# vovach777/llcomp

Hardware: AMD Instinct MI355X
Metric: encode+decode MPix/s on 4K RGB8, bit-exact (higher is better)
Workload: dtype int32

## Files before the change

llcomp_amd/csrc/enc_rows_asm.hpp:

```cpp
#pragma once
#include <cstdint>

namespace llcomp_mi {

#define LL_B0 "v32"
#define LL_B1 "v33"
#define LL_B "v[32:33]"
#define LL_A "v32"
#define LL_EX "v33"
#define LL_E0 "v[34:35]"
#define LL_E0L "v34"
#define LL_E0H "v35"
#define LL_E1 "v[36:37]"
#define LL_E1L "v36"
#define LL_E1H "v37"
#define LL_E2 "v[38:39]"
#define LL_E2L "v38"
#define LL_E2H "v39"
#define LL_E3 "v[40:41]"
#define LL_E3L "v40"
#define LL_E3H "v41"
#define LL_E4 "v[42:43]"
#define LL_E4L "v42"
#define LL_E4H "v43"
#define LL_E5 "v[44:45]"
#define LL_E5L "v44"
#define LL_E5H "v45"
#define LL_E6 "v[46:47]"
#define LL_E6L "v46"
#define LL_E6H "v47"
#define LL_E7 "v[48:49]"
#define LL_E7L "v48"
#define LL_E7H "v49"
#define LL_LOW "v30"
#define LL_RANGE "v31"
#define LL_LR "v[30:31]"
#define LL_R1 "v50"
#define LL_BITS "v51"
#define LL_N "v51"
#define LL_OFF "v52"
#define LL_T "v53"
#define LL_CK "v34"
#define LL_CT "v35"
#define LL_CT2 "v50"
#define LL_SX "s[36:37]"
#define LL_SA "s[38:39]"
#define LL_ST "s[40:41]"
#define LL_SW "s[42:43]"
#define LL_SB "s[44:45]"
#define LL_SU "s[46:47]"
#define LL_SM "s[56:57]"
#define LL_SC "s[40:41]"
#define LL_SD "s[48:49]"
#define LL_SE "s[50:51]"
#define LL_SR "s[52:53]"
#define LL_SRL "s52"
#define LL_SRH "s53"
#define LL_SI "s54"
#define LL_S1 "s52"
#define LL_S2 "s53"

#ifndef LLMI_ASM_VAR
#define LLMI_ASM_VAR 0
#endif
#if LLMI_ASM_VAR & 1
#define LL_C3 "3"
#else
#define LL_C3 "%[c3]"
#endif
#if LLMI_ASM_VAR & 4
#define LL_PATCH_SKIP(N)
#else
#define LL_PATCH_SKIP(N) "s_cbranch_execz .Lpatch" N "_%=\n\t"
#endif
#define LL_PATCH_END(N) ".Lpatch" N "_%=:\n\t" "s_mov_b64 exec, " LL_ST "\n\t"
#if LLMI_ASM_VAR & 2
#define LL_RENORM_SKIP(N)
#else
#define LL_RENORM_SKIP(N) "s_cbranch_execz .Lskip" N "_%=\n\t"
#endif
#define LL_SPLIT(EL)                                                                                              \
    "v_mul_u32_u24_sdwa " LL_R1 ", " EL ", " LL_RANGE " dst_sel:DWORD dst_unused:UNUSED_PAD src0_sel:BYTE_1 src1_sel:DWORD\n\t" \
    "v_lshrrev_b32_e32 " LL_R1 ", 8, " LL_R1 "\n\t"                                                               \
    "v_sub_u32_e32 " LL_RANGE ", " LL_RANGE ", " LL_R1 "\n\t"
#define LL_ONE                                          \
    "v_add_u32_e32 " LL_LOW ", " LL_LOW ", " LL_RANGE "\n\t"        \
    "v_mov_b32_e32 " LL_RANGE ", " LL_R1 "\n\t"
#define LL_RENORM(N)                                                                                               \
    "v_cmp_gt_u32_e32 vcc, %[c100], " LL_RANGE "\n\t"                                                                  \
    "s_and_saveexec_b64 " LL_SW ", vcc\n\t"                                                                        \
    LL_RENORM_SKIP(N)                                                                                              \
    "ds_write_b8_d16_hi %[wp], " LL_LOW "\n\t"                                                                         \
    "v_cmp_lt_u32_e32 vcc, %[cwrap], " LL_LOW "\n\t"                                                                   \
    "s_cbranch_vccnz .Lrare" N "_%=\n"                                                                             \
    ".Lback" N "_%=:\n\t"                                                                                          \
    "v_add_u32_e32 %[wp], 1, %[wp]\n\t"                                                                            \
    "v_lshlrev_b64 " LL_LR ", 8, " LL_LR "\n\t"                                                                     \
    "v_and_b32_e32 " LL_LOW ", 0xffffff, " LL_LOW "\n"                                                                     \
    ".Lskip" N "_%=:\n\t"                                                                                          \
    "s_mov_b64 exec, " LL_SW "\n\t"
#define LL_RARE_STUB(N)                     \
    ".Lrare" N "_%=:\n\t"                   \
    "s_getpc_b64 " LL_SR "\n\t"             \
    "s_branch .Lcarry_%=\n\t"               \
    "s_branch .Lback" N "_%=\n"
#define LL_FETCH_REST                                                                                                         \
    "v_lshlrev_b32_sdwa " LL_E1L ", " LL_C3 ", " LL_B0 " dst_sel:DWORD dst_unused:UNUSED_PAD src0_sel:DWORD src1_sel:BYTE_1\n\t"      \
    "v_lshlrev_b32_sdwa " LL_E2L ", " LL_C3 ", " LL_B0 " dst_sel:DWORD dst_unused:UNUSED_PAD src0_sel:DWORD src1_sel:BYTE_2\n\t"      \
    "v_lshlrev_b32_sdwa " LL_E3L ", " LL_C3 ", " LL_B0 " dst_sel:DWORD dst_unused:UNUSED_PAD src0_sel:DWORD src1_sel:BYTE_3\n\t"      \
    "v_lshlrev_b32_sdwa " LL_E4L ", " LL_C3 ", " LL_B1 " dst_sel:DWORD dst_unused:UNUSED_PAD src0_sel:DWORD src1_sel:BYTE_0\n\t"      \
    "ds_read_b64 " LL_E1 ", " LL_E1L "\n\t"                                                                                   \
    "ds_read_b64 " LL_E2 ", " LL_E2L "\n\t"                                                                                   \
    "ds_read_b64 " LL_E3 ", " LL_E3L "\n\t"                                                                                   \
    "ds_read_b64 " LL_E4 ", " LL_E4L "\n\t"                                                                                   \
    "v_lshlrev_b32_sdwa " LL_E5L ", " LL_C3 ", " LL_B1 " dst_sel:DWORD dst_unused:UNUSED_PAD src0_sel:DWORD src1_sel:BYTE_1\n\t"      \
    "v_lshlrev_b32_sdwa " LL_E6L ", " LL_C3 ", " LL_B1 " dst_sel:DWORD dst_unused:UNUSED_PAD src0_sel:DWORD src1_sel:BYTE_2\n\t"      \
    "v_lshlrev_b32_sdwa " LL_E7L ", " LL_C3 ", " LL_B1 " dst_sel:DWORD dst_unused:UNUSED_PAD src0_sel:DWORD src1_sel:BYTE_3\n\t"      \
    "ds_read_b64 " LL_E5 ", " LL_E5L "\n\t"                                                                                   \
    "ds_read_b64 " LL_E6 ", " LL_E6L "\n\t"                                                                                   \
    "ds_read_b64 " LL_E7 ", " LL_E7L "\n\t"

struct EncRowsExtra {
    uint32_t pend;
    uint32_t hot;
    uint32_t any_pend;
};

#define LL_SNAP 0
#include "enc_sample_asm.inc"
#undef LL_SNAP
#define LL_SNAP 1
#include "enc_sample_asm.inc"
#undef LL_SNAP

}
```

llcomp_amd/csrc/enc_sample_asm.inc:

```
#if LL_SNAP
#define LL_STATE(...)
#else
#define LL_STATE(...) __VA_ARGS__
#endif
#define LL_UNARY(K, KM1, EL, EH, N, SAVE)                  \
    LL_SPLIT(EL)                                           \
    LL_STATE("ds_write_b8 %[bank], " EL " offset:" K "\n\t") \
    "v_cmp_lt_u32_e32 vcc, " KM1 ", " LL_EX "\n\t"         \
    "s_and_b64 exec, exec, vcc\n\t"                        \
    SAVE                                                   \
    "s_cbranch_execz .Lunary_done_%=\n\t"                  \
    LL_ONE                                                 \
    LL_STATE("ds_write_b8 %[bank], " EH " offset:" K "\n\t") \
    LL_RENORM(N)
#if LL_SNAP
__device__ __forceinline__ void enc_snap_sample_asm(unsigned long long& low_range, uint32_t& wp, EncRowsExtra& x, uint32_t b0, uint32_t b1,
                                                    int res, uint32_t base) {
#else
__device__ __forceinline__ void enc_rows_sample_asm(unsigned long long& low_range, uint32_t& wp, EncRowsExtra& x, uint32_t bank,
                                                    int res, uint32_t base) {
#endif
    asm volatile(
        "s_mov_b64 " LL_SX ", exec\n\t"
        LL_STATE("ds_read2st64_b32 " LL_B ", %[bank] offset1:1\n\t")
        "s_cmp_lg_u32 %[hot], 0\n\t"
        "s_waitcnt lgkmcnt(0)\n\t"
        "v_lshlrev_b32_sdwa " LL_E0L ", " LL_C3 ", " LL_B0 " dst_sel:DWORD dst_unused:UNUSED_PAD src0_sel:DWORD src1_sel:BYTE_0\n\t"
        "ds_read_b64 " LL_E0 ", " LL_E0L "\n\t"
        "s_cbranch_scc0 .Lcold_%=\n\t"
        LL_FETCH_REST
        "s_waitcnt lgkmcnt(7)\n\t"
        "s_branch .Lzero_%=\n"
        ".Lcold_%=:\n\t"
        "s_waitcnt lgkmcnt(0)\n"
        ".Lzero_%=:\n\t"
        LL_SPLIT(LL_E0L)
        LL_STATE("ds_write_b8 %[bank], " LL_E0L "\n\t")
        "v_cmp_eq_u32_e32 vcc, 0, %[res]\n\t"
        "s_andn2_b64 " LL_SA ", exec, vcc\n\t"
        "s_and_saveexec_b64 " LL_ST ", vcc\n\t"
        LL_PATCH_SKIP("0")
        LL_ONE
        LL_STATE("ds_write_b8 %[bank], " LL_E0H "\n")
        LL_PATCH_END("0")
        LL_RENORM("0")
        "s_and_b64 exec, " LL_SA ", " LL_SA "\n\t"
        "s_cbranch_execz .Ldone_%=\n\t"
        "s_mov_b64 " LL_SB ", 0\n\t"
        "s_mov_b64 " LL_SM ", 0\n\t"
        "s_cmp_lg_u32 %[hot], 0\n\t"
        "s_cbranch_scc1 .Lhave_%=\n\t"
        LL_FETCH_REST
        ".Lhave_%=:\n\t"
        "v_sub_u32_e32 " LL_A ", 0, %[res]\n\t"
        "v_max_i32_e32 " LL_A ", %[res], " LL_A "\n\t"
        "v_ffbh_u32_e32 " LL_EX ", " LL_A "\n\t"
        "v_sub_u32_e32 " LL_EX ", 31, " LL_EX "\n\t"
        "s_waitcnt lgkmcnt(0)\n\t"
        LL_UNARY("1", "0", LL_E1L, LL_E1H, "1", "s_mov_b64 " LL_SB ", exec\n\t")
        LL_UNARY("2", "1", LL_E2L, LL_E2H, "2", "s_mov_b64 " LL_SM ", exec\n\t")
        LL_UNARY("3", "2", LL_E3L, LL_E3H, "3", "")
        "s_mov_b64 " LL_SU ", exec\n\t"
        "v_add_u32_e32 " LL_N ", -3, " LL_EX "\n\t"
        "s_mov_b32 " LL_SI ", 0\n\t"
        ".p2align 6\n"
        ".Ltail_%=:\n\t"
        LL_SPLIT(LL_E4L)
        "v_cmp_lt_u32_e32 vcc, " LL_SI ", " LL_N "\n\t"
        "s_and_b64 exec, exec, vcc\n\t"
        "s_cbranch_execz .Ltail_done_%=\n\t"
        "v_lshrrev_b32_e32 " LL_OFF ", 16, " LL_E4H "\n\t"
        "ds_read_b64 " LL_E4 ", " LL_OFF "\n\t"
        LL_ONE
        LL_RENORM("4")
        "s_add_i32 " LL_SI ", " LL_SI ", 1\n\t"
        "s_waitcnt lgkmcnt(0)\n\t"
        "s_branch .Ltail_%=\n"
        ".Ltail_done_%=:\n\t"
        "s_mov_b64 exec, " LL_SU "\n\t"
        LL_STATE("ds_write_b8 %[bank], " LL_E4L " offset:256\n")
        ".Lunary_done_%=:\n\t"
        "s_mov_b64 exec, " LL_SA "\n\t"
        LL_RENORM("5")
        "s_and_b64 exec, " LL_SB ", " LL_SB "\n\t"
        "s_cbranch_execz .Lsign_%=\n\t"
        LL_SPLIT(LL_E5L)
        LL_STATE("ds_write_b8 %[bank], " LL_E5L " offset:257\n\t")
        "v_lshl_or_b32 " LL_BITS ", " LL_A ", 1, 1\n\t"
        "v_sub_u32_e32 " LL_T ", 31, " LL_EX "\n\t"
        "v_lshlrev_b32_e32 " LL_BITS ", " LL_T ", " LL_BITS "\n\t"
        "v_add_co_u32_e32 " LL_BITS ", vcc, " LL_BITS ", " LL_BITS "\n\t"
        "s_and_saveexec_b64 " LL_ST ", vcc\n\t"
        LL_PATCH_SKIP("5")
        LL_ONE
        LL_STATE("ds_write_b8 %[bank], " LL_E5H " offset:257\n")
        LL_PATCH_END("5")
        LL_RENORM("6")
        ".p2align 6\n"
        ".Lman_%=:\n\t"
        "v_cmp_ne_u32_e32 vcc, %[sent], " LL_BITS "\n\t"
        "s_and_b64 exec, exec, vcc\n\t"
        "s_cbranch_execz .Lman_done_%=\n\t"
        "v_add_co_u32_e32 " LL_BITS ", vcc, " LL_BITS ", " LL_BITS "\n\t"
        "s_waitcnt lgkmcnt(0)\n\t"
        LL_SPLIT(LL_E6L)
        "v_lshrrev_b32_e32 " LL_OFF ", 16, " LL_E6L "\n\t"
        "s_and_saveexec_b64 " LL_ST ", vcc\n\t"
        LL_PATCH_SKIP("6")
        LL_ONE
        "v_lshrrev_b32_e32 " LL_OFF ", 16, " LL_E6H "\n"
        LL_PATCH_END("6")
        "ds_read_b64 " LL_E6 ", " LL_OFF "\n\t"
        LL_RENORM("7")
        "s_branch .Lman_%=\n"
        LL_RARE_STUB("0") LL_RARE_STUB("1") LL_RARE_STUB("2") LL_RARE_STUB("3") LL_RARE_STUB("4")
        LL_RARE_STUB("5") LL_RARE_STUB("6") LL_RARE_STUB("7") LL_RARE_STUB("8")
        ".Lcarry_%=:\n\t"
        "s_and_saveexec_b64 " LL_SC ", vcc\n\t"
        "v_add_u32_e32 " LL_CK ", -1, %[wp]\n"
        ".Lcloop_%=:\n\t"
        "v_cmp_lt_u32_e32 vcc, " LL_CK ", %[base]\n\t"
        "s_and_b64 " LL_SD ", exec, vcc\n\t"
        "s_cbranch_scc0 .Lcin_%=\n\t"
        "s_mov_b64 " LL_SE ", exec\n\t"
        "s_mov_b64 exec, " LL_SD "\n\t"
        "v_mov_b32_e32 %[pend], 1\n\t"
        "s_mov_b32 %[anyp], 1\n\t"
        "s_andn2_b64 exec, " LL_SE ", " LL_SD "\n\t"
        "s_cbranch_execz .Lcdone_%=\n"
        ".Lcin_%=:\n\t"
        "ds_read_u8 " LL_CT ", " LL_CK "\n\t"
        "s_waitcnt lgkmcnt(0)\n\t"
        "v_add_u32_e32 " LL_CT2 ", 1, " LL_CT "\n\t"
        "ds_write_b8 " LL_CK ", " LL_CT2 "\n\t"
        "v_add_u32_e32 " LL_CK ", -1, " LL_CK "\n\t"
        "v_cmp_eq_u32_e32 vcc, 0xff, " LL_CT "\n\t"
        "s_and_b64 exec, exec, vcc\n\t"
        "s_cbranch_execnz .Lcloop_%=\n"
        ".Lcdone_%=:\n\t"
        "s_mov_b64 exec, " LL_SC "\n\t"
        "v_and_b32_e32 " LL_LOW ", 0xffffff, " LL_LOW "\n\t"
        "s_add_u32 " LL_SRL ", " LL_SRL ", 4\n\t"
        "s_addc_u32 " LL_SRH ", " LL_SRH ", 0\n\t"
        "s_setpc_b64 " LL_SR "\n"
        ".Lman_done_%=:\n\t"
        "s_mov_b64 exec, " LL_SM "\n\t"
        LL_STATE("v_lshrrev_b32_e32 " LL_T ", 3, " LL_OFF "\n\t")
        LL_STATE("ds_write_b8 %[bank], " LL_T " offset:258\n")
        ".Lsign_%=:\n\t"
        "s_mov_b64 exec, " LL_SA "\n\t"
        LL_SPLIT(LL_E7L)
        LL_STATE("ds_write_b8 %[bank], " LL_E7L " offset:259\n\t")
        "v_cmp_gt_i32_e32 vcc, 0, %[res]\n\t"
        "s_and_saveexec_b64 " LL_ST ", vcc\n\t"
        LL_PATCH_SKIP("7")
        LL_ONE
        LL_STATE("ds_write_b8 %[bank], " LL_E7H " offset:259\n")
        LL_PATCH_END("7")
        LL_RENORM("8")
        ".Ldone_%=:\n\t"
        "s_bcnt1_i32_b64 " LL_S1 ", " LL_SA "\n\t"
        "s_bcnt1_i32_b64 " LL_S2 ", " LL_SX "\n\t"
        "s_lshl_b32 " LL_S1 ", " LL_S1 ", 1\n\t"
        "s_cmp_ge_u32 " LL_S1 ", " LL_S2 "\n\t"
        "s_cselect_b32 %[hot], 1, 0\n\t"
        "s_mov_b64 exec, " LL_SX "\n\t"
#if LL_SNAP
        : "+{v[30:31]}"(low_range), [wp] "+v"(wp), [pend] "+v"(x.pend), [hot] "+s"(x.hot), [anyp] "+s"(x.any_pend), "+{v32}"(b0), "+{v33}"(b1)
        : [res] "v"(res),
#else
        : "+{v[30:31]}"(low_range), [wp] "+v"(wp), [pend] "+v"(x.pend), [hot] "+s"(x.hot), [anyp] "+s"(x.any_pend)
        : [bank] "v"(bank), [res] "v"(res),
#endif
          [base] "v"(base), [c100] "s"(0x100u), [cwrap] "s"(0xFFFFFFu),
          [sent] "s"(0x80000000u), [c3] "v"(3u)
        : "vcc", "scc", "memory",
#if !LL_SNAP
          "v32", "v33",
#endif
          "v34", "v35", "v36", "v37", "v38", "v39", "v40", "v41", "v42", "v43", "v44",
          "v45", "v46", "v47", "v48", "v49", "v50", "v51", "v52", "v53", "s36", "s37", "s38", "s39", "s40", "s41", "s42", "s43",
          "s44", "s45", "s46", "s47", "s48", "s49", "s50", "s51", "s52", "s53", "s54", "s56", "s57");
}


#undef LL_STATE
#undef LL_UNARY
```

llcomp_amd/csrc/slice_kernels.hip:

```cpp
#include <algorithm>
#include <type_traits>

#include "device_common.hpp"
#include "kernels.hpp"

#ifndef LLMI_ASM_ENC
#define LLMI_ASM_ENC 1
#endif
#if LLMI_ASM_ENC
#include "enc_rows_asm.hpp"
#endif
#ifndef LLMI_ASM_DEC
#define LLMI_ASM_DEC 1
#endif
#if LLMI_ASM_DEC
#include "dec_rows_asm.hpp"
#endif

namespace llcomp_mi {

namespace {

#ifdef LLMI_CLOCK_PROBE
constexpr uint32_t kProbeSlots = 1u << 15;
// ... 9 lines not shown
        if (threadIdx.x == 0) {
            g_probe[kernel][blockIdx.x & (kProbeSlots - 1)][0] = t1 - t;
            g_probe[kernel][blockIdx.x & (kProbeSlots - 1)][1] = r1 - r;
        }
    }
};
#define LLMI_PROBE_START() ProbeStamp probe_stamp; probe_stamp.start()
#define LLMI_PROBE_STOP(kernel) probe_stamp.stop(kernel)
__device__ unsigned long long g_probe_parts[kProbeSlots][4];
struct PartClock {
    unsigned long long acc[4] = {0, 0, 0, 0}, last;
    __device__ __forceinline__ void start() { last = __builtin_amdgcn_s_memtime(); }
    __device__ __forceinline__ void lap(int part) {
        const unsigned long long now = __builtin_amdgcn_s_memtime();
        acc[part] += now - last;
        last = now;
    }
    __device__ __forceinline__ void flush() {
        if (threadIdx.x == 0)
            for (int k = 0; k < 4; ++k) g_probe_parts[blockIdx.x & (kProbeSlots - 1)][k] = acc[k];
    }
};
#define LLMI_PARTS_DECL() PartClock part_clock
#define LLMI_PARTS_START() part_clock.start()
#define LLMI_PARTS_LAP(part) part_clock.lap(part)
#define LLMI_PARTS_FLUSH() part_clock.flush()
#else
#define LLMI_PROBE_START() do {} while (0)
#define LLMI_PROBE_STOP(kernel) do {} while (0)
#define LLMI_PARTS_DECL() do {} while (0)
#define LLMI_PARTS_START() do {} while (0)
#define LLMI_PARTS_LAP(part) do {} while (0)
#define LLMI_PARTS_FLUSH() do {} while (0)
#endif

using entry_t = unsigned long long;
struct EntryTable {
    entry_t v[128];
};
constexpr EntryTable make_entries() {
    EntryTable t{};
    for (uint32_t s = 0; s < 128; ++s) t.v[s] = entry_t(entry_lo(s)) | (entry_t(entry_hi(s)) << 32);
    return t;
}
__constant__ EntryTable c_entries = make_entries();

using lds_u8_ptr = __attribute__((address_space(3))) uint8_t*;
using lds_entry_ptr = const __attribute__((address_space(3))) unsigned long long*;
__device__ __forceinline__ uint32_t lds_address(const void* p) { return uint32_t(uintptr_t((lds_u8_ptr) reinterpret_cast<const uint8_t*>(p))); }
__device__ __forceinline__ void load_table(entry_t* tab) {
    const unsigned long long rebase = (unsigned long long)lds_address(tab) * 0x0001000000010000ull;
    for (uint32_t i = threadIdx.x; i < 128; i += blockDim.x) tab[i] = c_entries.v[i] + rebase;
    __syncthreads();
}
__device__ __forceinline__ entry_t lds_entry(uint32_t address) { return *reinterpret_cast<lds_entry_ptr>(uintptr_t(address)); }

__device__ __forceinline__ void drain_vector_memory() { __builtin_amdgcn_s_waitcnt(0x0F70); }

__device__ __forceinline__ uint32_t byte_of(uint32_t w, int k) { return (w >> (8 * k)) & 0xFF; }
__device__ __forceinline__ uint32_t consume_here(uint32_t v);
template <int SLOT>
__device__ __forceinline__ uint32_t slot_state(const uint32_t* bank) {
    return byte_of(bank[SLOT >> 2], SLOT & 3);
}
template <int SLOT>
__device__ __forceinline__ void set_slot_state(uint32_t* bank, uint32_t ns) {
    constexpr int W = SLOT >> 2, SH = (SLOT & 3) * 8;
    bank[W] = (bank[W] & ~(0xFFu << SH)) | (ns << SH);
}
struct Bank {
    uint32_t w[4];
    uint8_t* lds;
};
constexpr uint32_t kRowBankWords = 3 * 2 * 64;
[[maybe_unused]] __device__ __forceinline__ constexpr uint32_t rowbank_byte(int slot) { return uint32_t(slot >> 2) * 256u + uint32_t(slot & 3); }
constexpr uint32_t kWideBankWords = 3 * 4 * 64;
__device__ __forceinline__ constexpr uint32_t widebank_byte(int slot) { return uint32_t(slot >> 1) * 256u + uint32_t(slot & 1) * 2u; }
template <int SLOT>
__device__ __forceinline__ uint32_t wide_offset(const uint32_t (&w)[4]) {
    return (SLOT & 1) ? (w[SLOT >> 1] >> 16) : (w[SLOT >> 1] & 0xFFFFu);
}
template <int SLOT, bool INLDS>
__device__ __forceinline__ void put_state(Bank& b, uint32_t ns) {
    if constexpr (INLDS) b.lds[rowbank_byte(SLOT)] = uint8_t(ns);
    else set_slot_state<SLOT>(b.w, ns & 0xFF);
}
__device__ __forceinline__ uint32_t prob_of(entry_t e) { return byte_of(uint32_t(e), 1); }
__device__ __forceinline__ uint32_t successor(entry_t e, bool bit) { return bit ? uint32_t(e >> 32) : uint32_t(e); }

struct Entries {
    entry_t e0, e1, e2, e3, e4, e5, e6, e7;
    template <int SLOT>
    __device__ __forceinline__ entry_t get() const {
        if constexpr (SLOT == 0) return e0;
        else if constexpr (SLOT == 1) return e1;
        else if constexpr (SLOT == 2) return e2;
        else if constexpr (SLOT == 3) return e3;
        else if constexpr (SLOT == 4) return e4;
        else if constexpr (SLOT == 5) return e5;
        else if constexpr (SLOT == 6) return e6;
        else return e7;
    }
};
__device__ __forceinline__ void fetch_slot0(Entries& E, const uint32_t* bank, const entry_t* tab) {
    E.e0 = tab[slot_state<0>(bank)];
}
__device__ __forceinline__ void fetch_rest(Entries& E, const uint32_t* bank, const entry_t* tab) {
    E.e1 = tab[slot_state<1>(bank)];
    E.e2 = tab[slot_state<2>(bank)];
    E.e3 = tab[slot_state<3>(bank)];
    E.e4 = tab[slot_state<4>(bank)];
    E.e5 = tab[slot_state<5>(bank)];
    E.e6 = tab[slot_state<6>(bank)];
    E.e7 = tab[slot_state<7>(bank)];
}

__device__ __forceinline__ entry_t entry_at(const entry_t*, uint32_t nx) { return lds_entry(nx >> 16); }

__device__ __forceinline__ void publish_count(unsigned long long* counters, uint32_t which, uint32_t mine) {
    if (!counters) return;
    unsigned long long live = __ballot(mine != 0);
    if (live == 0) return;
    unsigned long long sum = 0;
    const unsigned long long all = __ballot(1);
    while (live) {
        const int lane = __builtin_ctzll(live);
        sum += uint32_t(__builtin_amdgcn_readlane(mine, lane));
        live &= live - 1;
    }
    if (threadIdx.x == uint32_t(__builtin_ctzll(all))) atomicAdd(counters + which, sum);
}

constexpr int kModelSmall = 0;
constexpr int kModelLarge = 1;
constexpr std::integral_constant<int, kModelSmall> no_model{};

struct RangeEnc {
    uint32_t low;
    uint32_t range;
    uint32_t wp;
    uint32_t base;
    uint8_t* area;
    int32_t flushed;
    uint8_t* out;
    uint8_t* gout;
    uint32_t oofs;
    uint32_t ostep;
    int32_t cap;
    uint32_t shift;
    uint32_t carries;
};
constexpr int kStageBytes = 32;
constexpr int kStagePad = 16;
__device__ __forceinline__ int32_t enc_pos(const RangeEnc& e) { return e.flushed + int32_t(e.wp - e.base); }
__device__ __forceinline__ uint8_t* unit_byte(RangeEnc& e, uint32_t k) {
    return e.out + ((size_t(k >> 4) << (e.shift + 4)) + (k & 15));
}
__device__ __forceinline__ void enc_flush16(RangeEnc& e) {
    uint32_t* a = reinterpret_cast<uint32_t*>(e.area);
    uint4 v, rest;
    v.x = a[0]; v.y = a[1]; v.z = a[2]; v.w = a[3];
    rest.x = a[4]; rest.y = a[5]; rest.z = a[6]; rest.w = a[7];
    if (e.flushed + 16 <= e.cap) *reinterpret_cast<uint4*>(e.gout + e.oofs) = v;
    e.oofs += e.ostep;
    a[0] = rest.x; a[1] = rest.y; a[2] = rest.z; a[3] = rest.w;
    e.flushed += 16;
    e.wp -= 16;
}
__device__ __forceinline__ void enc_carry_back(RangeEnc& e) {
    for (int32_t k = enc_pos(e) - 1; k >= 0; --k) {
        uint32_t v;
        if (k >= e.flushed) {
            uint8_t& r = e.area[k - e.flushed];
            v = r;
            r = uint8_t(v + 1);
        } else if (k < e.cap) {
            uint8_t* g = unit_byte(e, uint32_t(k));
            if (k == e.flushed - 1) ++e.carries;
            v = *g;
            *g = uint8_t(v + 1);
        } else {
            break;
        }
        if (v != 0xFF) break;
    }
}
__device__ __forceinline__ void enc_renorm(RangeEnc& e) {
    if (e.range < 0x100) {
        asm volatile("ds_write_b8_d16_hi %0, %1" : : "v"(e.wp), "v"(e.low) : "memory");
        const bool wrapped = e.low > 0xFFFFFFu;
        if (__builtin_expect(__builtin_amdgcn_ballot_w64(wrapped) != 0, 0)) {
            if (wrapped) enc_carry_back(e);
        }
        ++e.wp;
        asm("v_lshlrev_b32_sdwa %0, %1, %2 dst_sel:DWORD dst_unused:UNUSED_PAD src0_sel:DWORD src1_sel:WORD_0"
            : "=v"(e.low) : "v"(8u), "v"(e.low));
        e.range <<= 8;
    }
}
__device__ __forceinline__ void enc_core(RangeEnc& e, uint32_t P, uint32_t m) {
    const uint32_t r1 = __umul24(e.range, P) >> 8;
    const uint32_t r0 = e.range - r1;
    e.low += r0 & m;
    asm("v_bfi_b32 %0, %1, %2, %3" : "=v"(e.range) : "v"(m), "v"(r1), "v"(r0));
    enc_renorm(e);
}
__device__ __forceinline__ uint32_t successor_m(entry_t e, uint32_t m) {
    uint32_t r;
    asm("v_bfi_b32 %0, %1, %2, %3" : "=v"(r) : "v"(m), "v"(uint32_t(e >> 32)), "v"(uint32_t(e)));
    return r;
}
__device__ __forceinline__ uint32_t enc_step_msb(RangeEnc& e, uint32_t& bits, entry_t cur) {
    uint32_t off, r1;
    unsigned long long saved_exec;
    asm("v_add_co_u32_e32 %[bits], vcc, %[bits], %[bits]\n\t"
        "v_mul_u32_u24_sdwa %[r1], %[lo], %[range] dst_sel:DWORD dst_unused:UNUSED_PAD src0_sel:BYTE_1 src1_sel:DWORD\n\t"
        "v_lshrrev_b32_e32 %[r1], 8, %[r1]\n\t"
        "v_sub_u32_e32 %[range], %[range], %[r1]\n\t"
        "v_lshrrev_b32_e32 %[off], 16, %[lo]\n\t"
        "s_and_saveexec_b64 %[save], vcc\n\t"
        "v_add_u32_e32 %[low], %[low], %[range]\n\t"
        "v_mov_b32_e32 %[range], %[r1]\n\t"
        "v_lshrrev_b32_e32 %[off], 16, %[hi]\n\t"
        "s_mov_b64 exec, %[save]"
        : [bits] "+v"(bits), [range] "+v"(e.range), [low] "+v"(e.low), [off] "=&v"(off), [r1] "=&v"(r1), [save] "=&s"(saved_exec)
        : [lo] "v"(uint32_t(cur)), [hi] "v"(uint32_t(cur >> 32))
        : "vcc");
    enc_renorm(e);
    return off;
}
template <int SLOT, bool INLDS>
__device__ __forceinline__ void enc_once_m(RangeEnc& e, Bank& bank, const Entries& E, uint32_t m) {
    enc_core(e, prob_of(E.get<SLOT>()), m);
    put_state<SLOT, INLDS>(bank, successor_m(E.get<SLOT>(), m));
}
template <int SLOT, bool INLDS>
__device__ __forceinline__ void enc_once(RangeEnc& e, Bank& bank, const Entries& E, bool bit) {
    const entry_t en = E.get<SLOT>();
    const uint32_t r1 = __umul24(e.range, prob_of(en)) >> 8;
    if constexpr (INLDS) {
        e.range -= r1;
        put_state<SLOT, true>(bank, uint32_t(en));
        if (bit) {
            asm volatile("" : "+v"(e.low));
            e.low += e.range;
            e.range = r1;
            put_state<SLOT, true>(bank, uint32_t(en >> 32));
        }
        enc_renorm(e);
    } else {
        const uint32_t r0 = e.range - r1;
        e.low += bit ? r0 : 0u;
        e.range = bit ? r1 : r0;
        const uint32_t ns = successor(en, bit);
        enc_renorm(e);
        put_state<SLOT, INLDS>(bank, ns);
    }
}

template <bool ALL, bool INLDS>
__device__ __forceinline__ void enc_residual(RangeEnc& e, Bank& bank, const entry_t* tab, int res) {
    Entries E;
    fetch_slot0(E, bank.w, tab);
    if (ALL) fetch_rest(E, bank.w, tab);
    enc_once<0, INLDS>(e, bank, E, res == 0);
    if (res != 0) {
        if (!ALL) fetch_rest(E, bank.w, tab);
        const uint32_t a = uint32_t(res < 0 ? -res : res);
        const int ex = 31 - __clz(int(a));
        enc_once<1, INLDS>(e, bank, E, ex > 0);
        if (ex > 0) {
            enc_once<2, INLDS>(e, bank, E, ex > 1);
            if (ex > 1) {
                enc_once<3, INLDS>(e, bank, E, ex > 2);
                if (ex > 2) {
                    entry_t cur = E.e4;
                    const uint32_t ones = uint32_t(ex - 3);
                    uint32_t r1 = __umul24(e.range, prob_of(cur)) >> 8;
                    e.range -= r1;
                    for (uint32_t i = 0; i < ones; ++i) {
                        cur = entry_at(tab, uint32_t(cur >> 32));
                        e.low += e.range;
                        e.range = r1;
                        enc_renorm(e);
                        r1 = __umul24(e.range, prob_of(cur)) >> 8;
                        e.range -= r1;
                    }
                    enc_renorm(e);
                    put_state<4, INLDS>(bank, uint32_t(cur));
                }
            }
            enc_once_m<5, INLDS>(e, bank, E, uint32_t(__builtin_amdgcn_sbfe(int(a), uint32_t(ex - 1), 1u)));
            if (ex > 1) {
                entry_t cur = E.e6;
                uint32_t nx;
                uint32_t bits = ((a << 1) | 1u) << (32 - ex);
                do {
                    nx = enc_step_msb(e, bits, cur);
                    cur = lds_entry(nx);
                } while (bits != 0x80000000u);
                put_state<6, INLDS>(bank, (nx - lds_address(tab)) >> 3);
            }
        }
        enc_once<7, INLDS>(e, bank, E, res < 0);
    }
}

__device__ __forceinline__ void enc_finish_and_count(RangeEnc& e, int32_t& n_bytes) {
    e.range = 0xFF; e.low += 0xFF; enc_renorm(e);
    e.range = 0xFF; enc_renorm(e);
    n_bytes = enc_pos(e);
    while (int32_t(e.wp - e.base) > 0) enc_flush16(e);
}

extern __shared__ __attribute__((aligned(32))) unsigned char dyn_lds[];
constexpr uint32_t kRowsEncTabOff = 0, kRowsEncStageOff = 1024, kRowsEncBankOff = 1024 + 16 + 32 * 64;
constexpr uint32_t kRowsEncLdsBytes = kRowsEncBankOff + 3 * 64 * 8;
[[maybe_unused]] __device__ __forceinline__ void enc_carry_back_flushed(RangeEnc& e, uint8_t* out) {
    if (e.flushed > 0 && e.flushed - 1 < e.cap) ++e.carries;
    for (int32_t k = e.flushed - 1; k >= 0; --k) {
        if (k >= e.cap) break;
        uint8_t* g = out + ((size_t(uint32_t(k) >> 4) << (e.shift + 4)) + (uint32_t(k) & 15));
        const uint32_t v = *g;
        *g = uint8_t(v + 1);
        if (v != 0xFF) break;
    }
}
template <bool LDSTAB>
__device__ __forceinline__ void clear_lds_states() {
    if constexpr (LDSTAB) {
        unsigned long long* t = reinterpret_cast<unsigned long long*>(dyn_lds);
        for (uint32_t i = threadIdx.x; i < uint32_t(kContexts); i += blockDim.x) t[i] = 0;
    }
}
template <int NCH, bool ROWS, typename SYM, bool LDSTAB = false, bool SNAP = false, bool SEG = false, bool SMALL = false>
__global__ __launch_bounds__(64, ROWS ? 8 : 1) void k_encode_slices(const Geometry g, const uint32_t lpw,
                                                      const SYM* __restrict__ sym, uint64_t* __restrict__ states,
                                                      uint8_t* __restrict__ scratch, uint32_t* __restrict__ slice_len,
                                                      uint64_t* __restrict__ group_sum, uint32_t* status, const uint64_t gpat,
                                                      unsigned long long* __restrict__ counters, const uint32_t seg_first = 0,
                                                      uint32_t* __restrict__ seg_state = nullptr) {
    static_assert(!(SNAP && (ROWS || LDSTAB)) && (SNAP || !SEG), "one kernel family at a time");
    static_assert(!SMALL || (ROWS && sizeof(SYM) == 1), "the model is a template flag only where the kernel forms the contexts");
    constexpr bool ASM = (ROWS || SNAP) && LLMI_ASM_ENC != 0;
    entry_t* tab;
    uint8_t* stage;
    uint32_t* rowbank;
    if constexpr (ASM) {
        static_assert(kStagePad == 16 && kStageBytes == 32, "kRowsEncBankOff");
#ifdef LLMI_TEST_LDS_OFFSET
        __shared__ uint32_t s_displace[4];
        if (threadIdx.x < 4) reinterpret_cast<volatile uint32_t*>(s_displace)[threadIdx.x] = gpat != 0;
#endif
        tab = reinterpret_cast<entry_t*>(dyn_lds + kRowsEncTabOff);
        stage = dyn_lds + kRowsEncStageOff;
        rowbank = reinterpret_cast<uint32_t*>(dyn_lds + kRowsEncBankOff);
        if (uint32_t(uintptr_t((lds_u8_ptr)dyn_lds)) != 0) {
            if (threadIdx.x == 0) atomicOr(status, kStInternal);
            return;
        }
    } else {
        __shared__ entry_t s_tab[128];
        __shared__ __attribute__((aligned(32))) uint8_t s_stage[kStagePad + kStageBytes * 64];
        __shared__ uint32_t s_rowbank[ROWS ? kRowBankWords : 1];
        tab = s_tab;
        stage = s_stage;
        rowbank = s_rowbank;
    }
    clear_lds_states<LDSTAB>();
    load_table(tab);
    const uint32_t id = blockIdx.x * lpw + threadIdx.x;
    if (threadIdx.x >= lpw || id >= g.n_slices) return;
    const SliceRect r = slice_rect(g, id);
    RangeEnc e;
    e.low = 0; e.range = 0xFF00;
    e.flushed = 0;
    e.area = stage + kStagePad + threadIdx.x * kStageBytes;
    e.base = uint32_t(uintptr_t((lds_u8_ptr)stage)) + kStagePad + threadIdx.x * kStageBytes;
    e.wp = e.base - 1;
    e.out = scratch + ((((size_t(id >> g.lane_shift) * (g.slice_cap >> 4)) << g.lane_shift) + (id & ((1u << g.lane_shift) - 1))) << 4);
    e.gout = scratch + (((size_t(__builtin_amdgcn_readfirstlane(id >> g.lane_shift)) * (g.slice_cap >> 4)) << g.lane_shift) << 4);
    e.oofs = (id & ((1u << g.lane_shift) - 1)) << 4;
    e.ostep = 16u << g.lane_shift;
    asm volatile("" : "+v"(e.ostep));
    e.cap = int32_t(g.slice_cap);
    e.shift = g.lane_shift;
    e.carries = 0;
    const uint32_t n_row = r.sw * (NCH ? uint32_t(NCH) : g.nch);
    const SYM* p0 = sym + lane_order_index(g, id, 0);
    const size_t GW = size_t(1) << g.lane_shift;
    const uint32_t total = n_row * r.sh;
    bool hot = false;
    LLMI_PROBE_START();

    if constexpr (SNAP) {
        const uint32_t cap = snapshot_cap(g);
        const uint32_t grp = __builtin_amdgcn_readfirstlane(id >> g.lane_shift);
        const char* const gres = reinterpret_cast<const char*>(sym) + ((size_t(grp) * cap * 2) << g.lane_shift);
        const char* const gbank = reinterpret_cast<const char*>(states) + ((size_t(grp) * cap * 8) << g.lane_shift);
        const uint32_t row = 32u << g.lane_shift;
        uint32_t lofs = (id & ((1u << g.lane_shift) - 1)) * 32u;
        asm volatile("" : "+v"(lofs));
        auto load_res = [&](uint32_t i) -> int {
            i = min(i, cap - 1);
            return *reinterpret_cast<const int16_t*>(gres + size_t(i >> 4) * row + ((i & 15u) << 1) + lofs);
        };
        auto load_bank = [&](uint32_t i) -> uint2 {
            i = min(i, cap - 1);
            return *reinterpret_cast<const uint2*>(gbank + size_t(i >> 3) * (2 * row) + ((i & 7u) << 3) + 2 * lofs);
        };
        uint32_t i = 0, end = total;
        [[maybe_unused]] uint32_t* const rec = SEG ? seg_state + size_t(id) * 16 : nullptr;
        if constexpr (SEG) {
            if (seg_first >= total) return;
            i = seg_first;
            end = min(total, seg_first + kSnapMaxSamples);
            if (seg_first) {
                const uint4 a = *reinterpret_cast<const uint4*>(rec), b = *reinterpret_cast<const uint4*>(rec + 4);
                const uint4 s0 = *reinterpret_cast<const uint4*>(rec + 8), s1 = *reinterpret_cast<const uint4*>(rec + 12);
                e.low = a.x; e.range = a.y; e.wp = e.base + a.z; e.flushed = int32_t(a.w);
                e.carries = b.x; hot = b.y != 0;
                e.oofs += (uint32_t(e.flushed) >> 4) * e.ostep;
                uint32_t* const st = reinterpret_cast<uint32_t*>(e.area);
                st[0] = s0.x; st[1] = s0.y; st[2] = s0.z; st[3] = s0.w; st[4] = s1.x; st[5] = s1.y; st[6] = s1.z; st[7] = s1.w;
            }
        }
#if LLMI_ASM_ENC
        EncRowsExtra xs{0u, 0u, 0u};
        unsigned long long low_range = e.low | ((unsigned long long)e.range << 32);
#endif
        auto code = [&](int res, uint2 bk) {
#if LLMI_ASM_ENC
            enc_snap_sample_asm(low_range, e.wp, xs, bk.x, bk.y, res, e.base);
            if (__builtin_expect(xs.any_pend != 0, 0)) {
                xs.any_pend = 0;
                if (xs.pend) enc_carry_back_flushed(e, e.out);
                xs.pend = 0;
            }
#else
            Bank bank{{bk.x, bk.y}, nullptr};
            if (hot) enc_residual<true, false>(e, bank, tab, res); else enc_residual<false, false>(e, bank, tab, res);
            hot = __builtin_amdgcn_readfirstlane(2 * __popcll(__ballot(res != 0)) >= __popcll(__ballot(true)));
#endif
        };
        const uint32_t todo = end - i, todo0 = __builtin_amdgcn_readfirstlane(todo);
        const bool same = __builtin_amdgcn_ballot_w64(todo != todo0) == 0;
        const uint32_t n_bulk = i + (same ? todo0 & ~3u : 0);
        int r0 = load_res(i), r1 = load_res(i + 1), r2 = load_res(i + 2), r3 = load_res(i + 3);
        uint2 b0 = load_bank(i), b1 = load_bank(i + 1), b2 = load_bank(i + 2), b3 = load_bank(i + 3);
#define LLMI_SNAP_SAMPLE(R, B, AHEAD)                          \
        {                                                          \
            const int rc = int(consume_here(uint32_t(R)));        \
            uint2 bc = B;                                          \
            bc.x = consume_here(bc.x);                             \
            R = load_res(i + AHEAD);                               \
            B = load_bank(i + AHEAD);                              \
            if (e.wp >= e.base + 16) enc_flush16(e);               \
            code(rc, bc);                                          \
        }
        for (; i < n_bulk; i += 4) {
            LLMI_SNAP_SAMPLE(r0, b0, 4)
            LLMI_SNAP_SAMPLE(r1, b1, 5)
            LLMI_SNAP_SAMPLE(r2, b2, 6)
            LLMI_SNAP_SAMPLE(r3, b3, 7)
        }
        for (; i < end; ++i) {
            LLMI_SNAP_SAMPLE(r0, b0, 4)
            {
                const int tr = r0;
                const uint2 tb = b0;
                r0 = r1; r1 = r2; r2 = r3; r3 = tr;
                b0 = b1; b1 = b2; b2 = b3; b3 = tb;
            }
        }
#undef LLMI_SNAP_SAMPLE
#if LLMI_ASM_ENC
        e.low = uint32_t(low_range);
        e.range = uint32_t(low_range >> 32);
#endif
        if constexpr (SEG) {
            if (end < total) {
                const uint32_t* const st = reinterpret_cast<const uint32_t*>(e.area);
                *reinterpret_cast<uint4*>(rec) = make_uint4(e.low, e.range, e.wp - e.base, uint32_t(e.flushed));
                *reinterpret_cast<uint4*>(rec + 4) = make_uint4(e.carries, hot ? 1u : 0u, 0u, 0u);
                *reinterpret_cast<uint4*>(rec + 8) = make_uint4(st[0], st[1], st[2], st[3]);
                *reinterpret_cast<uint4*>(rec + 12) = make_uint4(st[4], st[5], st[6], st[7]);
                return;
            }
        }
    } else if constexpr (ROWS) {
        for (uint32_t k = 0; k < 6; ++k) rowbank[k * 64 + threadIdx.x] = 0;
        constexpr bool PX = sizeof(SYM) == 1;
        const char* gsym;
        uint32_t sofs, sstep;
        [[maybe_unused]] uint32_t n_dword = total;
        [[maybe_unused]] uint32_t psh = 0, msub = 0, my = 0;
        [[maybe_unused]] int pl = 128, pL = 128;
        if constexpr (PX) {
            const uint32_t C = g.c;
            const unsigned long long tbase = ((unsigned long long)(r.frame) * g.h + r.y0) * g.w * C + (unsigned long long)(r.x0) * C;
            const unsigned long long wbase = (unsigned long long)uint32_t(__builtin_amdgcn_readfirstlane(uint32_t(tbase))) |
                                             ((unsigned long long)uint32_t(__builtin_amdgcn_readfirstlane(uint32_t(tbase >> 32))) << 32);
            gsym = reinterpret_cast<const char*>(sym) + wbase;
            sofs = uint32_t(tbase - wbase);
            sstep = C;
            const unsigned long long total_bytes = (unsigned long long)(g.frames) * g.h * g.w * C;
            n_dword = rows_px_dwords(tbase, total, C, total_bytes);
            psh = 8 * r.ch;
            msub = C >= 3 && (r.ch == 0 || r.ch == 2) ? ~0u : 0u;
            my = C >= 3 && r.ch == 1 ? ~0u : 0u;
            asm volatile("" : "+v"(psh), "+v"(msub), "+v"(my));
        } else {
            const uint32_t grp = __builtin_amdgcn_readfirstlane(id >> g.lane_shift);
            gsym = reinterpret_cast<const char*>(sym + ((size_t(grp) * g.slice_samples) << g.lane_shift));
            sofs = (id & ((1u << g.lane_shift) - 1)) * uint32_t(sizeof(SYM));
            sstep = uint32_t(sizeof(SYM)) << g.lane_shift;
        }
        asm volatile("" : "+v"(sstep));
        auto load_sym = [&](uint32_t ofs) -> uint32_t {
            if constexpr (PX) {
                uint32_t w;
                __builtin_memcpy(&w, gsym + ofs, 4);
                return w;
            } else {
                return *reinterpret_cast<const SYM*>(gsym + ofs);
            }
        };
        auto load_at = [&](uint32_t ofs, uint32_t k) -> uint32_t {
            if constexpr (PX) {
                if (k >= n_dword) {
                    const uint8_t* p = reinterpret_cast<const uint8_t*>(gsym + ofs);
                    uint32_t w = p[0];
                    if (g.c > 1) w |= uint32_t(p[1]) << 8;
                    if (g.c > 2) w |= uint32_t(p[2]) << 16;
                    if (g.c > 3) w |= uint32_t(p[3]) << 24;
                    return w;
                }
            }
            return load_sym(ofs);
        };
        uint32_t s0 = load_at(sofs, 0);
        sofs += sstep;
        uint32_t s1 = total > 1 ? load_at(sofs, 1) : 0;
        sofs += sstep;
        uint32_t bank_base = uint32_t(uintptr_t((lds_u8_ptr) reinterpret_cast<uint8_t*>(rowbank))) + threadIdx.x * 4;
        asm volatile("" : "+v"(bank_base));
#if LLMI_ASM_ENC
        EncRowsExtra xs{0u, 0u, 0u};
        unsigned long long low_range = e.low | ((unsigned long long)e.range << 32);
#endif
        auto front = [&](uint32_t sy) -> uint32_t {
            uint32_t t = sy;
            if constexpr (PX) {
                const uint32_t G = (sy >> 8) & 0xFF;
                const int sum = int(sy & 0xFF) + int((sy >> 16) & 0xFF) - 2 * int(G);
                const int q = (sum + int((uint32_t(sum) >> 31) * 3u)) >> 2;
                t = uint32_t(int(__builtin_amdgcn_ubfe(sy, psh, 8)) - int(G & msub) + (q & int(my)));
            }
            asm volatile("" : "+v"(t) : : "memory");
            return t;
        };
        struct Ctx {
            uint32_t bofs;
            int sg;
        };
        auto context = [&](auto model) -> Ctx {
            constexpr int MODEL = decltype(model)::value;
            Ctx c{0u, 0};
            if constexpr (PX && MODEL != kModelSmall) {
                const int dq = pL - pl;
                c.sg = dq >> 31;
                asm volatile("" : "+v"(c.sg));
                const uint32_t aq = uint32_t((dq ^ c.sg) - c.sg);
                c.bofs = ((aq + 511u) & 0x200u) + ((aq + 508u) & 0x200u);
                asm volatile("" : "+v"(c.bofs));
            }
            return c;
        };
        auto code = [&](uint32_t sy, Ctx c, auto model) {
            constexpr int MODEL = decltype(model)::value;
            uint32_t bofs = c.bofs;
            int res;
            if constexpr (PX) {
                const int v = int(sy);
                res = MODEL == kModelSmall ? v - pl : ((v - pl) ^ c.sg) - c.sg;
                pL = pl;
                pl = v;
            } else if constexpr (sizeof(SYM) == 2) {
                bofs = (sy >> 3) & 0x600u;
                res = int(sy << 20) >> 20;
            } else {
                bofs = (((sy & 0xFFFF) * 109u) >> 7) & 0x600u;
                res = int(sy) >> 16;
            }
#if LLMI_ASM_ENC
            enc_rows_sample_asm(low_range, e.wp, xs, bank_base + bofs, res, e.base);
            if (__builtin_expect(xs.any_pend != 0, 0)) {
                xs.any_pend = 0;
                if (xs.pend) enc_carry_back_flushed(e, e.gout + (size_t(id & ((1u << g.lane_shift) - 1)) << 4));
                xs.pend = 0;
            }
#else
            uint32_t* bp = reinterpret_cast<uint32_t*>(reinterpret_cast<uint8_t*>(rowbank) + threadIdx.x * 4 + bofs);
            Bank bank{{bp[0], bp[64]}, reinterpret_cast<uint8_t*>(bp)};
            if (hot) enc_residual<true, true>(e, bank, tab, res); else enc_residual<false, true>(e, bank, tab, res);
            hot = __builtin_amdgcn_readfirstlane(2 * __popcll(__ballot(res != 0)) >= __popcll(__ballot(true)));
#endif
        };
        const uint32_t total0 = __builtin_amdgcn_readfirstlane(total);
        const bool same = __builtin_amdgcn_ballot_w64(total != total0) == 0;
        const uint32_t tail = PX ? rows_px_tail(g.c) : 2u;
        const uint32_t n_bulk = same && total0 > tail ? total0 - tail : 0;
        auto sample_tested = [&](uint32_t i, auto model) {
            s0 = consume_here(s0);
            const Ctx c0 = context(model);
            const uint32_t t0 = front(s0);
            const uint32_t s2 = i + 2 < total ? load_at(sofs, i + 2) : 0;
            sofs += sstep;
            if (e.wp >= e.base + 16) enc_flush16(e);
            code(t0, c0, model);
            s0 = s1;
            s1 = s2;
        };
        auto bulk = [&](uint32_t& i, auto model) {
            for (; i + 1 < n_bulk; i += 2) {
                s0 = consume_here(s0);
                const Ctx c0 = context(model);
                const uint32_t t0 = front(s0);
                s0 = load_sym(sofs);
                sofs += sstep;
                if (e.wp >= e.base + 16) enc_flush16(e);
                code(t0, c0, model);
                s1 = consume_here(s1);
                const Ctx c1 = context(model);
                const uint32_t t1 = front(s1);
                s1 = load_sym(sofs);
                sofs += sstep;
                if (e.wp >= e.base + 16) enc_flush16(e);
                code(t1, c1, model);
            }
            for (; i < total; ++i) sample_tested(i, model);
        };
        sample_tested(0, no_model);
        if (total > 1) sample_tested(1, no_model);
#if LLMI_ASM_ENC
        xs.hot = __builtin_amdgcn_readfirstlane(xs.hot);
        xs.any_pend = 0;
#endif
        uint32_t i = 2;
        bulk(i, std::integral_constant<int, SMALL ? kModelSmall : kModelLarge>{});
#if LLMI_ASM_ENC
        e.low = uint32_t(low_range);
        e.range = uint32_t(low_range >> 32);
#endif
    } else {
        uint64_t* banks;
        uint32_t bsh;
        if constexpr (LDSTAB) {
            banks = reinterpret_cast<uint64_t*>(dyn_lds);
            bsh = 0;
        } else {
            banks = states + ((size_t(id >> g.lane_shift) * kContexts) << g.lane_shift) + (id & ((1u << g.lane_shift) - 1));
            bsh = g.lane_shift;
        }
        uint32_t fk = 0;
        auto fetch = [&]() -> uint32_t { return p0[size_t(fk++) * GW]; };
        uint32_t s0 = fetch();
        uint32_t s1 = total > 1 ? fetch() : 0;
        uint64_t b0 = bank_fresh<LDSTAB>(banks[size_t(s0 & 0xFFFF) << bsh], gpat);
        for (uint32_t i = 0; i < total; ++i) {
            const uint32_t s2 = i + 2 < total ? fetch() : 0;
            const uint32_t ctx0 = s0 & 0xFFFF, ctx1 = s1 & 0xFFFF;
            const int res = int(s0) >> 16;
            uint64_t raw1 = (i + 1 < total) ? banks[size_t(ctx1) << bsh] : 0;
            Bank bank{{uint32_t(b0), uint32_t(b0 >> 32)}, nullptr};
            if (hot) enc_residual<true, false>(e, bank, tab, res); else enc_residual<false, false>(e, bank, tab, res);
            hot = __builtin_amdgcn_readfirstlane(2 * __popcll(__ballot(res != 0)) >= __popcll(__ballot(true)));
            b0 = uint64_t(bank.w[0]) | (uint64_t(bank.w[1]) << 32);
            if constexpr (!LDSTAB) drain_vector_memory();
            uint64_t b1 = bank_fresh<LDSTAB>(raw1, gpat);
            banks[size_t(ctx0) << bsh] = bank_tagged<LDSTAB>(b0, gpat);
            if (ctx1 == ctx0) b1 = b0;
            b0 = b1;
            if (e.wp >= e.base + 16) enc_flush16(e);
            s0 = s1;
            s1 = s2;
        }
    }
    int32_t n_bytes = enc_pos(e);
    enc_finish_and_count(e, n_bytes);
    LLMI_PROBE_STOP(0);
    if (n_bytes > e.cap) {
        atomicOr(status, kStOverflow);
        n_bytes = e.cap;
    }
    slice_len[id] = uint32_t(n_bytes);
    publish_count(counters, kCtrEncCarryBacks, e.carries);
    if (group_sum) {
        unsigned long long live = __ballot(1), sum = 0;
        while (live) {
            const int lane = __builtin_ctzll(live);
            sum += uint32_t(__builtin_amdgcn_readlane(n_bytes, lane));
            live &= live - 1;
        }
        if (threadIdx.x == 0) group_sum[blockIdx.x] = sum;
    }
}

template <int SLOT, bool INLDS>
__device__ __forceinline__ void dec_put_state(Bank& b, uint32_t half) {
    if constexpr (INLDS) *reinterpret_cast<uint16_t*>(b.lds + widebank_byte(SLOT)) = uint16_t(half >> 16);
    else set_slot_state<SLOT>(b.w, half & 0xFF);
}
template <int SLOT, bool INLDS>
__device__ __forceinline__ entry_t dec_entry(const Bank& b, const entry_t* tab) {
    if constexpr (INLDS) return lds_entry(wide_offset<SLOT>(b.w));
    else return tab[slot_state<SLOT>(b.w)];
}
template <bool INLDS>
__device__ __forceinline__ void dec_fetch_slot0(Entries& E, const Bank& b, const entry_t* tab) { E.e0 = dec_entry<0, INLDS>(b, tab); }
template <bool INLDS>
__device__ __forceinline__ void dec_fetch_rest(Entries& E, const Bank& b, const entry_t* tab) {
    E.e1 = dec_entry<1, INLDS>(b, tab);
    E.e2 = dec_entry<2, INLDS>(b, tab);
    E.e3 = dec_entry<3, INLDS>(b, tab);
    E.e4 = dec_entry<4, INLDS>(b, tab);
    E.e5 = dec_entry<5, INLDS>(b, tab);
    E.e6 = dec_entry<6, INLDS>(b, tab);
    E.e7 = dec_entry<7, INLDS>(b, tab);
}
struct RangeDec {
    uint32_t low, range;
    unsigned long long win;
    uint32_t nxt;
    const char* gbase;
    uint32_t ofs;
    uint32_t step;
    uint32_t ofs_end;
    uint32_t replays;
};
__device__ __forceinline__ bool window_low(const RangeDec& d) { return uint32_t(d.win >> 32) == 0; }
__device__ __forceinline__ void dec_prefetch(RangeDec& d) {
    d.nxt = *reinterpret_cast<const uint32_t*>(d.gbase + min(d.ofs, d.ofs_end));
    d.ofs += d.step;
}
__device__ __forceinline__ uint32_t consume_here(uint32_t v) {
    asm volatile("" : "+v"(v) : : "memory");
    return v;
}
__device__ __forceinline__ void dec_append(RangeDec& d) {
    const uint32_t ready = consume_here(d.nxt);
    const uint32_t sh = 31u - uint32_t(__builtin_clz(uint32_t(d.win)));
    const uint32_t rest = uint32_t(d.win) ^ (1u << sh);
    d.win = ((0x100000000ull | ready) << sh) | rest;
    dec_prefetch(d);
}
__device__ __forceinline__ void dec_append_drained(RangeDec& d) {
    dec_append(d);
    drain_vector_memory();
}
__device__ __forceinline__ void dec_open(RangeDec& d, const uint32_t* group, uint32_t lane, uint32_t shift, uint32_t len) {
    d.gbase = reinterpret_cast<const char*>(group);
    d.ofs = lane * 4;
    d.step = 4u << shift;
    asm volatile("" : "+v"(d.step));
    d.ofs_end = lane * 4 + ((len + 3) >> 2) * d.step;
    dec_prefetch(d);
    const uint32_t first = d.nxt;
    dec_prefetch(d);
    const unsigned long long both = first | ((unsigned long long)d.nxt << 32);
    dec_prefetch(d);
    d.range = 0xFF00;
    d.low = ((first & 0xFF) << 8) | ((first >> 8) & 0xFF);
    d.win = (both >> 16) | (1ull << 48);
    d.replays = 0;
}
__device__ __forceinline__ unsigned long long window_next(unsigned long long w) {
    unsigned long long r;
    asm("v_lshrrev_b64 %0, 8, %1" : "=v"(r) : "v"(w));
    return r;
}
__device__ __forceinline__ void dec_refill(RangeDec& d) {
    if (d.range < 0x100) {
        d.range <<= 8;
        d.low = (d.low << 8) | (uint32_t(d.win) & 0xFF);
        d.win = window_next(d.win);
    }
}
template <bool CHECKED>
__device__ __forceinline__ bool dec_core(RangeDec& d, uint32_t P) {
    if (CHECKED && d.win <= 1) dec_append_drained(d);
    const uint32_t r1 = __umul24(d.range, P) >> 8;
    const uint32_t r0 = d.range - r1;
    uint32_t diff;
    const bool under = __builtin_usub_overflow(d.low, r0, &diff);
    const bool bit = !under;
    d.low = under ? d.low : diff;
    d.range = under ? r0 : r1;
    dec_refill(d);
    return bit;
}
template <bool CHECKED>
__device__ __forceinline__ uint32_t dec_step_acc(RangeDec& d, uint32_t P, entry_t cur, uint32_t& w) {
    if (CHECKED && d.win <= 1) dec_append_drained(d);
    const uint32_t r1 = __umul24(d.range, P) >> 8;
    const uint32_t r0 = d.range - r1;
    uint32_t diff, nx;
    asm("v_sub_co_u32_e32 %[diff], vcc, %[low], %[r0]\n\t"
        "s_nop 1\n\t"
        "v_cndmask_b32_e32 %[range], %[r1], %[r0], vcc\n\t"
        "v_cndmask_b32_e32 %[low], %[diff], %[low], vcc\n\t"
        "v_cndmask_b32_e32 %[nx], %[hi], %[lo], vcc\n\t"
        "v_addc_co_u32_e32 %[w], vcc, %[w], %[w], vcc"
        : [diff] "=&v"(diff), [range] "=&v"(d.range), [low] "+v"(d.low), [nx] "=&v"(nx), [w] "+v"(w)
        : [r0] "v"(r0), [r1] "v"(r1), [lo] "v"(uint32_t(cur)), [hi] "v"(uint32_t(cur >> 32))
        : "vcc");
    if (d.range < 0x100) {
        d.range <<= 8;
        d.low = (d.low << 8) | (uint32_t(d.win) & 0xFF);
        d.win = window_next(d.win);
    }
    return nx;
}
template <int SLOT, bool CHECKED, bool INLDS>
__device__ __forceinline__ bool dec_once(RangeDec& d, Bank& bank, const Entries& E) {
    const entry_t en = E.get<SLOT>();
    const bool bit = dec_core<CHECKED>(d, prob_of(en));
    dec_put_state<SLOT, INLDS>(bank, successor(en, bit));
    return bit;
}
template <bool ALL, bool CHECKED, bool INLDS>
__device__ __forceinline__ bool dec_residual(RangeDec& d, Bank& bank, const entry_t* tab, uint32_t& out) {
    Entries E;
    dec_fetch_slot0<INLDS>(E, bank, tab);
    if (ALL) dec_fetch_rest<INLDS>(E, bank, tab);
    if (dec_once<0, CHECKED, INLDS>(d, bank, E)) {
        out = 0;
        return true;
    }
    if (!ALL) dec_fetch_rest<INLDS>(E, bank, tab);
    int ex = 0;
    bool ok = true;
    if (dec_once<1, CHECKED, INLDS>(d, bank, E)) {
// ... 531 lines not shown
```

Before: 28820.

## Use v_cmpx loop tests, batch staging flushes, and dot4 pixel transform

Replaces the cmp+s_and exec-narrowing pairs with single v_cmpx instructions and rotates the tail and mantissa loops so the test sits at the bottom. Batches the per-sample 16-byte staging flush behind a wave-uniform ballot with a higher threshold, so the flush branch is skipped most of the time, and adds a final flush at finish. Rewrites the RGB colour-decorrelation front end with udot4 instructions in place of several shifts and subtracts. The batched flush relies on the staging buffer having room for the extra bytes, which the new static_asserts check.

```diff
diff --git a/llcomp_amd/csrc/enc_rows_asm.hpp b/llcomp_amd/csrc/enc_rows_asm.hpp
--- a/llcomp_amd/csrc/enc_rows_asm.hpp
+++ b/llcomp_amd/csrc/enc_rows_asm.hpp
@@ -79,6 +79,7 @@
 #else
 #define LL_RENORM_SKIP(N) "s_cbranch_execz .Lskip" N "_%=\n\t"
 #endif
+#define LL_NARROW(OP, A, B) "v_cmpx_" OP "_e32 vcc, " A ", " B "\n\t"
 #define LL_SPLIT(EL)                                                                                              \
     "v_mul_u32_u24_sdwa " LL_R1 ", " EL ", " LL_RANGE " dst_sel:DWORD dst_unused:UNUSED_PAD src0_sel:BYTE_1 src1_sel:DWORD\n\t" \
     "v_lshrrev_b32_e32 " LL_R1 ", 8, " LL_R1 "\n\t"                                                               \
diff --git a/llcomp_amd/csrc/enc_sample_asm.inc b/llcomp_amd/csrc/enc_sample_asm.inc
--- a/llcomp_amd/csrc/enc_sample_asm.inc
+++ b/llcomp_amd/csrc/enc_sample_asm.inc
@@ -6,8 +6,7 @@
 #define LL_UNARY(K, KM1, EL, EH, N, SAVE)                  \
     LL_SPLIT(EL)                                           \
     LL_STATE("ds_write_b8 %[bank], " EL " offset:" K "\n\t") \
-    "v_cmp_lt_u32_e32 vcc, " KM1 ", " LL_EX "\n\t"         \
-    "s_and_b64 exec, exec, vcc\n\t"                        \
+    LL_NARROW("lt_u32", KM1, LL_EX)                        \
     SAVE                                                   \
     "s_cbranch_execz .Lunary_done_%=\n\t"                  \
     LL_ONE                                                 \
@@ -63,19 +62,20 @@
         "s_mov_b64 " LL_SU ", exec\n\t"
         "v_add_u32_e32 " LL_N ", -3, " LL_EX "\n\t"
         "s_mov_b32 " LL_SI ", 0\n\t"
+        LL_SPLIT(LL_E4L)
+        LL_NARROW("lt_u32", LL_SI, LL_N)
+        "s_cbranch_execz .Ltail_done_%=\n\t"
         ".p2align 6\n"
         ".Ltail_%=:\n\t"
-        LL_SPLIT(LL_E4L)
-        "v_cmp_lt_u32_e32 vcc, " LL_SI ", " LL_N "\n\t"
-        "s_and_b64 exec, exec, vcc\n\t"
-        "s_cbranch_execz .Ltail_done_%=\n\t"
         "v_lshrrev_b32_e32 " LL_OFF ", 16, " LL_E4H "\n\t"
         "ds_read_b64 " LL_E4 ", " LL_OFF "\n\t"
         LL_ONE
         LL_RENORM("4")
         "s_add_i32 " LL_SI ", " LL_SI ", 1\n\t"
         "s_waitcnt lgkmcnt(0)\n\t"
-        "s_branch .Ltail_%=\n"
+        LL_SPLIT(LL_E4L)
+        LL_NARROW("lt_u32", LL_SI, LL_N)
+        "s_cbranch_execnz .Ltail_%=\n"
         ".Ltail_done_%=:\n\t"
         "s_mov_b64 exec, " LL_SU "\n\t"
         LL_STATE("ds_write_b8 %[bank], " LL_E4L " offset:256\n")
@@ -96,11 +96,10 @@
         LL_STATE("ds_write_b8 %[bank], " LL_E5H " offset:257\n")
         LL_PATCH_END("5")
         LL_RENORM("6")
+        LL_NARROW("ne_u32", "%[sent]", LL_BITS)
+        "s_cbranch_execz .Lman_done_%=\n\t"
         ".p2align 6\n"
         ".Lman_%=:\n\t"
-        "v_cmp_ne_u32_e32 vcc, %[sent], " LL_BITS "\n\t"
-        "s_and_b64 exec, exec, vcc\n\t"
-        "s_cbranch_execz .Lman_done_%=\n\t"
         "v_add_co_u32_e32 " LL_BITS ", vcc, " LL_BITS ", " LL_BITS "\n\t"
         "s_waitcnt lgkmcnt(0)\n\t"
         LL_SPLIT(LL_E6L)
@@ -112,7 +111,9 @@
         LL_PATCH_END("6")
         "ds_read_b64 " LL_E6 ", " LL_OFF "\n\t"
         LL_RENORM("7")
-        "s_branch .Lman_%=\n"
+        LL_NARROW("ne_u32", "%[sent]", LL_BITS)
+        "s_cbranch_execnz .Lman_%=\n\t"
+        "s_branch .Lman_done_%=\n"
         LL_RARE_STUB("0") LL_RARE_STUB("1") LL_RARE_STUB("2") LL_RARE_STUB("3") LL_RARE_STUB("4")
         LL_RARE_STUB("5") LL_RARE_STUB("6") LL_RARE_STUB("7") LL_RARE_STUB("8")
         ".Lcarry_%=:\n\t"
diff --git a/llcomp_amd/csrc/slice_kernels.hip b/llcomp_amd/csrc/slice_kernels.hip
--- a/llcomp_amd/csrc/slice_kernels.hip
+++ b/llcomp_amd/csrc/slice_kernels.hip
@@ -185,6 +185,11 @@
 };
 constexpr int kStageBytes = 32;
 constexpr int kStagePad = 16;
+constexpr int kSampleBytesMax = 13;
+constexpr int kFlushAt = 19;
+constexpr int kStageFill = kFlushAt - 1 + kSampleBytesMax;
+static_assert(kStageFill <= kStageBytes - 1, "the staging area's last byte belongs to the next lane's dummy byte");
+static_assert(kStageFill - 16 <= kFlushAt - 1 && kFlushAt >= 16, "one unit per lane and flush event must be enough");
 __device__ __forceinline__ int32_t enc_pos(const RangeEnc& e) { return e.flushed + int32_t(e.wp - e.base); }
 __device__ __forceinline__ uint8_t* unit_byte(RangeEnc& e, uint32_t k) {
     return e.out + ((size_t(k >> 4) << (e.shift + 4)) + (k & 15));
@@ -199,6 +204,13 @@
     a[0] = rest.x; a[1] = rest.y; a[2] = rest.z; a[3] = rest.w;
     e.flushed += 16;
     e.wp -= 16;
+}
+__device__ __forceinline__ void enc_flush_batched(RangeEnc& e) {
+    if (__builtin_amdgcn_ballot_w64(e.wp >= e.base + uint32_t(kFlushAt)) != 0) {
+        uint32_t w = e.wp + uint32_t(kFlushAt - 16);
+        asm volatile("" : "+v"(w));
+        if (w >= e.base + uint32_t(kFlushAt)) enc_flush16(e);
+    }
 }
 __device__ __forceinline__ void enc_carry_back(RangeEnc& e) {
     for (int32_t k = enc_pos(e) - 1; k >= 0; --k) {
@@ -339,7 +351,11 @@
     }
 }
 
+template <bool BATCHED>
 __device__ __forceinline__ void enc_finish_and_count(RangeEnc& e, int32_t& n_bytes) {
+    if constexpr (BATCHED) {
+        if (e.wp >= e.base + 16) enc_flush16(e);
+    }
     e.range = 0xFF; e.low += 0xFF; enc_renorm(e);
     e.range = 0xFF; enc_renorm(e);
     n_bytes = enc_pos(e);
@@ -527,7 +543,7 @@
         const char* gsym;
         uint32_t sofs, sstep;
         [[maybe_unused]] uint32_t n_dword = total;
-        [[maybe_unused]] uint32_t psh = 0, msub = 0, my = 0;
+        [[maybe_unused]] uint32_t xm = 0, coef = 0, my = 0;
         [[maybe_unused]] int pl = 128, pL = 128;
         if constexpr (PX) {
             const uint32_t C = g.c;
@@ -539,10 +555,12 @@
             sstep = C;
             const unsigned long long total_bytes = (unsigned long long)(g.frames) * g.h * g.w * C;
             n_dword = rows_px_dwords(tbase, total, C, total_bytes);
-            psh = 8 * r.ch;
-            msub = C >= 3 && (r.ch == 0 || r.ch == 2) ? ~0u : 0u;
+            const bool diff = C >= 3 && (r.ch == 0 || r.ch == 2);
+            xm = diff ? 0xFF00u : 0u;
+            coef = diff ? (r.ch == 0 ? 0x0101u : 0x010100u) : 1u << (8 * r.ch);
             my = C >= 3 && r.ch == 1 ? ~0u : 0u;
-            asm volatile("" : "+v"(psh), "+v"(msub), "+v"(my));
+            pl = pL = 128 + int(xm >> 8);
+            asm volatile("" : "+v"(xm), "+v"(coef), "+v"(my));
         } else {
             const uint32_t grp = __builtin_amdgcn_readfirstlane(id >> g.lane_shift);
             gsym = reinterpret_cast<const char*>(sym + ((size_t(grp) * g.slice_samples) << g.lane_shift));
@@ -585,10 +603,11 @@
         auto front = [&](uint32_t sy) -> uint32_t {
             uint32_t t = sy;
             if constexpr (PX) {
-                const uint32_t G = (sy >> 8) & 0xFF;
-                const int sum = int(sy & 0xFF) + int((sy >> 16) & 0xFF) - 2 * int(G);
-                const int q = (sum + int((uint32_t(sum) >> 31) * 3u)) >> 2;
-                t = uint32_t(int(__builtin_amdgcn_ubfe(sy, psh, 8)) - int(G & msub) + (q & int(my)));
+                const int sum = int(__builtin_amdgcn_udot4(sy ^ 0xFF00u, 0x010201u, uint32_t(-510), false));
+                int neg = sum >> 31;
+                asm volatile("" : "+v"(neg));
+                const int q = (sum + (neg & 3)) >> 2;
+                t = __builtin_amdgcn_udot4(sy ^ xm, coef, uint32_t(q & int(my)), false);
             }
             asm volatile("" : "+v"(t) : : "memory");
             return t;
@@ -650,7 +669,7 @@
             const uint32_t t0 = front(s0);
             const uint32_t s2 = i + 2 < total ? load_at(sofs, i + 2) : 0;
             sofs += sstep;
-            if (e.wp >= e.base + 16) enc_flush16(e);
+            enc_flush_batched(e);
             code(t0, c0, model);
             s0 = s1;
             s1 = s2;
@@ -662,14 +681,14 @@
                 const uint32_t t0 = front(s0);
                 s0 = load_sym(sofs);
                 sofs += sstep;
-                if (e.wp >= e.base + 16) enc_flush16(e);
+                enc_flush_batched(e);
                 code(t0, c0, model);
                 s1 = consume_here(s1);
                 const Ctx c1 = context(model);
                 const uint32_t t1 = front(s1);
                 s1 = load_sym(sofs);
                 sofs += sstep;
-                if (e.wp >= e.base + 16) enc_flush16(e);
+                enc_flush_batched(e);
                 code(t1, c1, model);
             }
             for (; i < total; ++i) sample_tested(i, model);
@@ -721,7 +740,7 @@
         }
     }
     int32_t n_bytes = enc_pos(e);
-    enc_finish_and_count(e, n_bytes);
+    enc_finish_and_count<ROWS>(e, n_bytes);
     LLMI_PROBE_STOP(0);
     if (n_bytes > e.cap) {
         atomicOr(status, kStOverflow);
```

Result: faster. 29530 (median of 6 runs) (+2.5%).
